# alexv879/ClusterMachineLearningForHospitalNetworks-Apache-Spark

Hardware: AMD Instinct MI355X
Metric: KMeans fit samples/sec (whole node), 100M×256 k=256 at 1/2/4/8 MI355X (higher is better)
Workload: dtype bf16; 1 GPU; model=KMeans k=256, 100000000x256, global_batch=100000000, parallelism=dp1, k=256, rows=100000000, dim=256

## Files before the change

### clustermachinelearningforhospitalnetworks_apache_spark_amd/_native/csrc/kmeans.hip

```cpp
#include <algorithm>

#include "common.h"

namespace {

constexpr int kAccumThreads = 1024;
constexpr int kSegThreads = 256;

template <int DP>
struct AssignShape {
  static constexpr int NCH = DP / 8;
  static constexpr int KS = DP >= 32 ? DP / 32 : 1;
};
constexpr int kAssignThreads = 512;

template <bool HI>
__device__ __forceinline__ unsigned f8x2_to_bf16x2(unsigned w) {
  typedef float f2 __attribute__((ext_vector_type(2)));
  const f2 v = __builtin_amdgcn_cvt_pk_f32_fp8((int)w, HI);
  return (__float_as_uint(v.x) >> 16) | (__float_as_uint(v.y) & 0xffff0000u);
}

template <int DP, bool F8>
__device__ __forceinline__ void load_x16(const void* __restrict__ Xv, long long n, long long ldx, long long row0,
// ... 512 lines not shown
      for (int u = 0; u < kScatterU; ++u) {
        rows[u] = (long long)b * grp + (q0 + (long long)u * per) * stride + o;
        lab[u] = rows[u] < n ? labels[rows[u]] : -1;
        rk[u] = rows[u] < n ? rank[rows[u]] : 0;
      }
#pragma unroll
      for (int u = 0; u < kScatterU; ++u)
        if (lab[u] >= 0) {
          const long long pos = (long long)soff[lab[u]] + rk[u];
          if (pos < n) perm[pos] = (int)rows[u];
        }
    }
  }
}

template <int CPL> struct RawCols;
template <> struct RawCols<2> { using T = unsigned; };
template <> struct RawCols<4> { using T = uint2; };
template <> struct RawCols<8> { using T = uint4; };

template <int CPL>
__device__ __forceinline__ void add_raw(double (&acc)[CPL], const typename RawCols<CPL>::T& w) {
  const unsigned* ws = reinterpret_cast<const unsigned*>(&w);
#pragma unroll
  for (int q = 0; q < CPL / 2; ++q) {
    acc[2 * q] += (double)bf16_to_f32((u16)(ws[q] & 0xffffu));
    acc[2 * q + 1] += (double)bf16_to_f32((u16)(ws[q] >> 16));
  }
}

template <int CPL>
__device__ __forceinline__ void add_raw_q(double (&acc)[CPL], const typename RawCols<CPL>::T& w, double qs,
                                          float qsf) {
  const unsigned* ws = reinterpret_cast<const unsigned*>(&w);
  if (qsf != 0.f) {
#pragma unroll
    for (int q = 0; q < CPL / 2; ++q) {
      acc[2 * q] += (double)rintf(bf16_to_f32((u16)(ws[q] & 0xffffu)) * qsf);
      acc[2 * q + 1] += (double)rintf(bf16_to_f32((u16)(ws[q] >> 16)) * qsf);
    }
  } else {
#pragma unroll
    for (int q = 0; q < CPL / 2; ++q) {
      acc[2 * q] += rint((double)bf16_to_f32((u16)(ws[q] & 0xffffu)) * qs);
      acc[2 * q + 1] += rint((double)bf16_to_f32((u16)(ws[q] >> 16)) * qs);
    }
  }
}

__device__ __forceinline__ float grid_scale_f32(double qs) {
  return (qs >= 0x1p-126 && qs <= 0x1p126) ? (float)qs : 0.f;
}

template <int CPL> struct RawCols8;
template <> struct RawCols8<4> { using T = unsigned; };
template <> struct RawCols8<8> { using T = uint2; };
template <> struct RawCols8<16> { using T = uint4; };

template <int CPL>
__device__ __forceinline__ void add_raw8(double (&acc)[CPL], const typename RawCols8<CPL>::T& w) {
  typedef float f2 __attribute__((ext_vector_type(2)));
  const unsigned* ws = reinterpret_cast<const unsigned*>(&w);
#pragma unroll
  for (int q = 0; q < CPL / 4; ++q) {
    const f2 a = __builtin_amdgcn_cvt_pk_f32_fp8((int)ws[q], false);
    const f2 b = __builtin_amdgcn_cvt_pk_f32_fp8((int)ws[q], true);
    acc[4 * q] += (double)a.x;
    acc[4 * q + 1] += (double)a.y;
    acc[4 * q + 2] += (double)b.x;
    acc[4 * q + 3] += (double)b.y;
  }
}

template <int CPL>
__device__ __forceinline__ void add_raw8_f32(float (&acc)[CPL], const typename RawCols8<CPL>::T& w) {
  typedef float f2 __attribute__((ext_vector_type(2)));
  const unsigned* ws = reinterpret_cast<const unsigned*>(&w);
#pragma unroll
  for (int q = 0; q < CPL / 4; ++q) {
    const f2 a = __builtin_amdgcn_cvt_pk_f32_fp8((int)ws[q], false);
    const f2 b = __builtin_amdgcn_cvt_pk_f32_fp8((int)ws[q], true);
    acc[4 * q] += a.x;
    acc[4 * q + 1] += a.y;
    acc[4 * q + 2] += b.x;
    acc[4 * q + 3] += b.y;
  }
}

template <int CPL, bool F8> struct SegRaw { using T = typename RawCols<CPL>::T; };
template <int CPL> struct SegRaw<CPL, true> { using T = typename RawCols8<CPL>::T; };

template <int CPL, bool F8>
__device__ __forceinline__ float sqdist_raw(const typename SegRaw<CPL, F8>::T& w, const float (&cv)[CPL]) {
  const unsigned* ws = reinterpret_cast<const unsigned*>(&w);
  float s = 0.f;
  if constexpr (F8) {
    typedef float f2 __attribute__((ext_vector_type(2)));
#pragma unroll
    for (int q = 0; q < CPL / 4; ++q) {
      const f2 a = __builtin_amdgcn_cvt_pk_f32_fp8((int)ws[q], false);
      const f2 b = __builtin_amdgcn_cvt_pk_f32_fp8((int)ws[q], true);
      const float e0 = a.x - cv[4 * q], e1 = a.y - cv[4 * q + 1], e2 = b.x - cv[4 * q + 2], e3 = b.y - cv[4 * q + 3];
      s = fmaf(e0, e0, s);
      s = fmaf(e1, e1, s);
      s = fmaf(e2, e2, s);
      s = fmaf(e3, e3, s);
    }
  } else {
#pragma unroll
    for (int q = 0; q < CPL / 2; ++q) {
      const float e0 = bf16_to_f32((u16)(ws[q] & 0xffffu)) - cv[2 * q];
      const float e1 = bf16_to_f32((u16)(ws[q] >> 16)) - cv[2 * q + 1];
      s = fmaf(e0, e0, s);
      s = fmaf(e1, e1, s);
    }
  }
  return s;
}

__device__ __forceinline__ float wave_total_dpp(float v) {
  v += __int_as_float(__builtin_amdgcn_update_dpp(0, __float_as_int(v), 0xB1, 0xf, 0xf, false));
  v += __int_as_float(__builtin_amdgcn_update_dpp(0, __float_as_int(v), 0x4E, 0xf, 0xf, false));
  v += __int_as_float(__builtin_amdgcn_update_dpp(0, __float_as_int(v), 0x141, 0xf, 0xf, false));
  v += __int_as_float(__builtin_amdgcn_update_dpp(0, __float_as_int(v), 0x140, 0xf, 0xf, false));
  v += __int_as_float(__builtin_amdgcn_update_dpp(0, __float_as_int(v), 0x142, 0xa, 0xf, false));
  v += __int_as_float(__builtin_amdgcn_update_dpp(0, __float_as_int(v), 0x143, 0xc, 0xf, false));
  return __int_as_float(__builtin_amdgcn_readlane(__float_as_int(v), 63));
}

__device__ __forceinline__ float batch16_totals(const float (&s)[16]) {
  const int lane = threadIdx.x & 63;
  const bool h5 = lane & 32, h4 = lane & 16, h3 = lane & 8, h2 = lane & 4;
  float a[8], b[4], c[2];
#pragma unroll
  for (int i = 0; i < 8; ++i) a[i] = (h5 ? s[8 + i] : s[i]) + __shfl_xor(h5 ? s[i] : s[8 + i], 32, 64);
#pragma unroll
  for (int i = 0; i < 4; ++i) b[i] = (h4 ? a[4 + i] : a[i]) + __shfl_xor(h4 ? a[i] : a[4 + i], 16, 64);
#pragma unroll
  for (int i = 0; i < 2; ++i) c[i] = (h3 ? b[2 + i] : b[i]) + __shfl_xor(h3 ? b[i] : b[2 + i], 8, 64);
  float v = (h2 ? c[1] : c[0]) + __shfl_xor(h2 ? c[0] : c[1], 4, 64);
  v += __int_as_float(__builtin_amdgcn_update_dpp(0, __float_as_int(v), 0xB1, 0xf, 0xf, false));
  v += __int_as_float(__builtin_amdgcn_update_dpp(0, __float_as_int(v), 0x4E, 0xf, 0xf, false));
  return __shfl(v, 4 * (lane & 15), 64);
}

struct SegUB {
  const u16* cb;
  long long ldc;
  float* ub;
  double qs;
  const float* cu = nullptr;
};

__device__ __forceinline__ long long seg_chunk(long long filled, long long waves) {
  const long long c = (filled + waves - 1) / waves;
  return c > 128 ? c : 128;
}

template <int CPL, bool F8, bool UB = false, bool Q = false>
__global__ __launch_bounds__(kSegThreads, (CPL <= 4 ? 4 : 1)) void kmeans_segacc(const void* __restrict__ X, long long n, long long ldx,
                                                             int Dp, int D, const int* __restrict__ perm,
                                                             const int* __restrict__ seg, int k,
                                                             double* __restrict__ msg, double* __restrict__ slots,
                                                             int* __restrict__ slot_c, const int* __restrict__ gate,
                                                             int want, SegUB sub) {
  using raw_t = typename SegRaw<CPL, F8>::T;
  constexpr int U = 16;
// ... 998 lines not shown
```

### clustermachinelearningforhospitalnetworks_apache_spark_amd/models/kmeans.py

```python
from __future__ import annotations

import math
import os
import types
from typing import List, Optional

import numpy as np
import torch

from .. import _native
from ..ops import kmeans_ops as K
from ..ops.group_ops import group_reduce
from ..parallel.comm import Communicator, local_comm
from ..utils import rng
from ..utils.device import padded_dim, round_up
from ..utils.fault import maybe_fail
from ..utils.trace import trace


def padded_dim_fp8(d: int) -> int:
    return max(256, 1 << max(0, (d - 1).bit_length()))


def to_device_matrix(x: torch.Tensor, d: Optional[int] = None) -> torch.Tensor:
# ... 906 lines not shown
        st.lb = torch.zeros(max(n, 1), dtype=torch.float32, device=dev)
        st.cb_old = torch.zeros_like(self.cb)
        st.cb_cost = torch.zeros_like(self.cb)
        st.cum = cum if lazy else None
        st.half_every = int(os.environ.get("CML_KMEANS_HALF_EVERY", "4"))
        st.replay = {} if os.environ.get("CML_KMEANS_REPLAY", "1") != "0" else None
        st.replay_refused = None
        st.pm_host = torch.zeros(1, dtype=torch.int32, pin_memory=True) if self.gpu else None
        self._pst = st
        if self._norms_ready:
            self._set_mx()
        lean = os.environ.get("CML_KMEANS_LEAN_STEP", "1") != "0" and not self.use_graph
        per_wg_all = -(-(-(-max(n, 1) // tr)) // ap.grid) * tr
        self.delta = K.DeltaState(max(n, 1), k, d, self.dp, 1, self.msg_len, dev, ap.grid, fp8=K.is_fp8(self.x),
                                  cap=max(st.cap_m, 1024), pcap=max(per_wg_all if lean else per_wg, 64), lean=lean)

    def _step_prune_dev(self) -> None:
        self._pdev_pre()
        self.comm.allreduce_async(self.msgs[0]).wait()
        self._pdev_post()

    def _pdev_pre(self) -> None:
        st, dl = self._pst, self.delta
        hint_full = int(st.pm_host[0]) != 0
        lean = dl.lean_step() and not hint_full
        if self._replay_ok():
            if self._replay(("pre", lean), lambda: self._pdev_pre_launches(lean)):
                dl.host_forced = False
                return
        self._pdev_pre_launches(lean)
# ... 20 lines not shown

    def _pdev_pre_launches(self, lean: bool) -> None:
        st, dl = self._pst, self.delta
        n, k, d, ap = self.n, self.k, self.d, self.aplan
        x, lab, msg = self.x, self.labels, self.msgs[0]
        K.prune_bounds_gated(lab[:n], st.ub, st.lb, st.drift, st.dmax, st.thr, st.c2, k, st.cand, st.count,
                             self.xnorm, st.cand_lab, st.cand_xn, st.flags, st.cum, st.pmode, st.cap_m,
                             st.backoff if st.nback > 0 else None, st.nback, st.ctr[0:1], mode_host=st.pm_host)
        K.assign_rr_ext(1, x, n, self.dp, self.cb, self.cnorm, ap, self.xnorm, lab, self.cost_part, st.ub, st.lb,
                        st.mc, st.tau, hist=self.hist, rank=self.rank, delta=dl, gate=st.pmode, want=1, cum=st.cum)
        K.assign_rr_ext(2, x, st.cap_m, self.dp, self.cb, self.cnorm, ap, st.cand_xn, lab, self.cost_part, st.ub,
                        st.lb, st.mc, st.tau, delta=dl, idx=st.cand, n_dev=st.count, lab_in=st.cand_lab,
                        gate=st.pmode, want=0, cum=st.cum)
        dl.gate(0, lean=lean)
        if not lean:
            K.accumulate_sort(x, n, self.dp, d, lab, self.rank, self.hist, ap, k, self.cost_part, self.off, self.seg,
                              self.perm, self.cplan, dl.acc[0], self.slots, gate=dl.mode[0], qscale=self._qscale)
        dl.accumulate(x, self.dp, lab, 0, self.cost_part, ap.grid, msg, qscale=self._qscale)

    def _replay_ok(self) -> bool:
        st = self._pst
        return (not self.use_graph and self._grid_done and st.replay is not None
                and not torch.cuda.is_current_stream_capturing())

    def _pdev_post(self) -> None:
        st = self._pst
        exact = self.use_graph or st.half_every <= 1 or self.iterations % st.half_every == 0
        if not (self._replay_ok() and not self.spherical and self.dp <= 2048
                and self._replay(("post", exact, self._conv_lim), lambda: self._pdev_post_launches(exact))):
            self._pdev_post_launches(exact)
        self._shift2 = self.shift2
        self._cost_fn = self._device_cost

# ... 31 lines not shown

    def _step_seeded(self) -> None:
        st, dl = self._pst, self.delta
        n, k, d, ap = self.n, self.k, self.d, self.aplan
        x, lab, msg = self.x, self.labels, self.msgs[0]
        if n:
            K.prune_bounds(lab, st.ub, st.lb, st.drift, st.dmax, st.thr, st.c2, k, st.cand, st.count,
                           xn=self.xnorm, cand_lab=st.cand_lab, cand_xn=st.cand_xn, zero_count=True, cum=st.cum)
            K.prune_gate(st.count, st.cap_m, st.flags, st.pmode)
            K.assign_rr_ext(1, x, n, self.dp, self.cb, self.cnorm, ap, self.xnorm, lab, self.cost_part, st.ub, st.lb,
                            st.mc, st.tau, hist=self.hist, rank=self.rank, delta=dl, gate=st.pmode, want=1,
                            cum=st.cum)
            K.assign_rr_ext(2, x, st.cap_m, self.dp, self.cb, self.cnorm, ap, st.cand_xn, lab, None, st.ub, st.lb,
                            st.mc, st.tau, delta=dl, idx=st.cand, n_dev=st.count, lab_in=st.cand_lab, gate=st.pmode,
                            want=0, cum=st.cum)
            K.label_hist(lab, n, ap, self.hist, self.rank, gate=st.pmode, want=0)
        self.cost_part.zero_()
        dl.invalidate()
        dl.gate(0)
        K.accumulate_sort(x, n, self.dp, d, lab, self.rank, self.hist, ap, k, self.cost_part, self.off, self.seg,
                          self.perm, self.cplan, dl.acc[0], self.slots, gate=dl.mode[0],
                          ub_centres=self.cb, ub=st.ub, qscale=self._qscale, cum=st.cum)
        dl.accumulate(x, self.dp, lab, 0, self.cost_part, ap.grid, msg, qscale=self._qscale)
        self.comm.allreduce_async(msg).wait()
        self._pdev_post()

    def _norms64(self) -> torch.Tensor:
        self._ensure_norms()
        if self._xnorm64 is None:
            self._xnorm64 = torch.empty(max(self.n, 1), dtype=torch.float64, device=self.device)
            if self.n:
                tmp = torch.empty(self.n, dtype=torch.float32, device=self.device)
                for _, r0, r1, xc in self._x_chunks(whole=True):
                    K.row_pass(xc, r1 - r0, self.dp, tmp[r0:r1], xn64=self._xnorm64[r0:r1])
        return self._xnorm64

    def _device_cost(self) -> torch.Tensor:
# ... 847 lines not shown
```

### clustermachinelearningforhospitalnetworks_apache_spark_amd/ops/kmeans_ops.py

```python
from __future__ import annotations

import ctypes
import os
import threading

from dataclasses import dataclass

import torch

from .. import _native
from .._native import c_dbl, c_int, c_ll, c_vp
from ..utils.device import LDS_BUDGET, num_cus, round_up

_native.register_kernel_sigs({
    "cml_kmeans_assign_lds_bytes": (c_ll, [c_int, c_int, c_int]),
    "cml_kmeans_assign_threads": (c_int, [c_int]),
    "cml_kmeans_set_assign_variant": (c_int, [c_int]),
    "cml_kmeans_assign_occupancy": (c_int, [c_int, c_int, c_int, c_int]),
    "cml_kmeans_seg_threads": (c_int, []),
    "cml_kmeans_seg_ints": (c_ll, [c_int]),
    "cml_kmeans_assign_bf16": (c_int, [c_vp, c_ll, c_ll, c_int, c_vp, c_ll, c_int, c_int, c_int, c_vp, c_vp, c_vp,
                                       c_vp, c_int, c_int, c_vp, c_vp, c_vp, c_int, c_int, c_vp, c_vp, c_vp, c_vp,
                                       c_int, c_int, c_vp]),
    "cml_kmeans_assign_rr_plan": (c_int, [c_int, c_int, c_int, c_int, c_vp]),
# ... 2 lines not shown
    "cml_kmeans_set_rr_m32": (c_int, [c_int]),
    "cml_kmeans_set_fp8_mx": (c_int, [c_int]),
    "cml_kmeans_assign_tile_rows": (c_int, [c_int]),
    "cml_row_sqnorm_bf16": (c_int, [c_vp, c_ll, c_ll, c_int, c_vp, c_vp]),
    "cml_row_sqnorm_fp8": (c_int, [c_vp, c_ll, c_ll, c_int, c_vp, c_vp]),
    "cml_kmeans_priv_lds_bytes": (c_ll, [c_int, c_int, c_int]),
    "cml_kmeans_accum_priv": (c_int, [c_vp, c_ll, c_ll, c_vp, c_int, c_int, c_int, c_int, c_vp, c_vp, c_int, c_int,
                                      c_vp]),
    "cml_kmeans_reduce": (c_int, [c_vp, c_vp, c_vp, c_int, c_int, c_int, c_int, c_int, c_vp, c_vp]),
    "cml_kmeans_sort_accum": (c_int, [c_vp, c_ll, c_ll, c_int, c_int, c_vp, c_vp, c_vp, c_int, c_int, c_int, c_int,
                                      c_vp, c_int, c_vp, c_vp, c_vp, c_int, c_int, c_vp, c_vp, c_vp, c_int, c_vp,
                                      ctypes.c_double, c_vp]),
    "cml_kmeans_sort_accum_ub": (c_int, [c_vp, c_ll, c_ll, c_int, c_int, c_vp, c_vp, c_vp, c_int, c_int, c_int,
                                         c_int, c_vp, c_int, c_vp, c_vp, c_vp, c_int, c_int, c_vp, c_vp, c_vp, c_int,
                                         c_vp, c_vp, c_ll, c_vp, ctypes.c_double, c_vp, c_vp]),
    "cml_kmeans_delta_gate": (c_int, [c_vp, c_int, c_int, c_vp, c_vp, c_vp, c_int, c_vp, c_vp]),
    "cml_kmeans_delta_accum": (c_int, [c_vp, c_ll, c_int, c_int, c_vp, c_vp, c_vp, c_vp, c_int, c_int, c_int, c_vp,
                                       c_int, c_vp, c_vp, c_vp, c_vp, c_int, c_int, c_vp, c_vp, c_vp, c_vp, c_vp,
                                       c_int, c_vp, c_int, ctypes.c_double, c_vp]),
    "cml_kmeans_seg_slot_doubles": (c_ll, [c_int, c_int]),
    "cml_kmeans_seg_slot_ints": (c_ll, [c_int]),
    "cml_kmeans_update": (c_int, [c_vp, c_int, c_ll, c_int, c_int, c_vp, c_vp, c_ll, c_int, c_int, c_vp, c_vp,
                                  ctypes.c_double, c_vp]),
    "cml_kmeans_prune_lower": (c_int, [c_vp, c_int, c_vp, c_vp, ctypes.c_float, ctypes.c_float, c_ll, c_vp, c_vp]),
    "cml_kmeans_prune_bounds": (c_int, [c_vp, c_vp, c_vp, c_vp, c_vp, c_vp, c_vp, c_int, c_ll, c_vp,
                                        c_vp, c_vp, c_vp, c_vp, c_vp, c_ll, c_vp, c_vp]),
    "cml_kmeans_prune_gate": (c_int, [c_vp, c_ll, c_vp, c_vp, c_vp, c_int, c_vp]),
    "cml_kmeans_converge_latch": (c_int, [c_vp, c_int, ctypes.c_double, c_vp, c_vp]),
    "cml_kmeans_cond_copy": (c_int, [c_vp, c_vp, c_ll, c_vp, c_vp, c_vp]),
    "cml_kmeans_seed_bounds": (c_int, [c_vp, c_vp, c_vp, c_vp, c_vp, c_vp, c_vp, c_vp, ctypes.c_float, c_ll,
# ... 485 lines not shown
    lib = _native.kernels()
    args = (x.data_ptr(), n, x.stride(0), dp, d, labels.data_ptr(), rank.data_ptr(), hist.data_ptr(), aplan.grid,
            aplan.round_rows, k, aplan.kp, cost_part.data_ptr(), aplan.grid, off.data_ptr(), seg.data_ptr(),
            perm.data_ptr(), plan.cpl, plan.seg_grid, msg.data_ptr(), slots[0].data_ptr(), slots[1].data_ptr(),
            int(is_fp8(x)), gate.data_ptr() if gate is not None else 0)
    if ub is not None:
        if ub_centres is None or ub_centres.dtype != torch.bfloat16 or ub.dtype != torch.float32 or ub.numel() < n:
            raise ValueError("accumulate_sort: ub needs bf16 centres and an f32 [n] output")
        status = lib.cml_kmeans_sort_accum_ub(*args, ub_centres.data_ptr(), ub_centres.stride(0), ub.data_ptr(),
                                              float(qscale), _ptr(cum), _native.stream_ptr(stream))
    else:
        status = lib.cml_kmeans_sort_accum(*args, float(qscale), _native.stream_ptr(stream))
    _native.check(status, "kmeans_sort_accum")


def sort_perm(labels: torch.Tensor, rank: torch.Tensor, hist: torch.Tensor, aplan: AssignPlan, n: int, k: int,
              off: torch.Tensor, seg: torch.Tensor, perm: torch.Tensor, tail: torch.Tensor | None = None,
              cost_part: torch.Tensor | None = None, stream=None) -> torch.Tensor:
    i32 = torch.int32
    if any(t.dtype != i32 or not t.is_contiguous() for t in (labels, rank, hist, off, seg, perm)):
        raise ValueError("sort_perm: contiguous int32 labels, rank, hist, off, seg and perm")
    if (labels.numel() < n or rank.numel() < n or perm.numel() < n or hist.numel() < aplan.grid * aplan.kp
            or off.numel() < k * aplan.grid or seg.numel() < seg_buffer_ints(k) or k > aplan.kp):
        raise ValueError("sort_perm: buffer lengths do not match n, k and the assign plan")
    if tail is None:
        tail = torch.empty(k + 1, dtype=torch.float64, device=labels.device)
    elif tail.dtype != torch.float64 or tail.numel() < k + 1 or not tail.is_contiguous():
        raise ValueError("sort_perm: tail is a contiguous f64 [k + 1] tensor")
    if cost_part is not None and (cost_part.dtype != torch.float64 or cost_part.numel() < aplan.grid):
        raise ValueError("sort_perm: cost_part is the assign's f64 [grid] tensor")
# ... 728 lines not shown
```

Baseline: 118.7 billion samples/s.

## Add row-block LDS bucketing accumulate kernel replacing global sort-based accumulate

Adds a new kmeans_blockacc kernel. Each workgroup takes a block of rows, counts their labels in LDS, bucket-sorts row indices locally, sums rows per centre into per-block f64 slabs, and optionally computes upper bounds in the same pass. This is meant to remove the global label histogram, sort and permutation passes of the sort-based accumulate. The trade-off is extra per-block slab storage and a reduction of those slabs, plus LDS pressure that limits occupancy. In auto mode it only runs when 80*k fits within the block row count, and the default path uses it for the upper-bound full accumulate while plain accumulates stay on the sort path unless the env var is set to 1.

After: 111.8 billion samples/s. 0.942x the previous value.

```diff
diff --git a/clustermachinelearningforhospitalnetworks_apache_spark_amd/_native/csrc/kmeans.hip b/clustermachinelearningforhospitalnetworks_apache_spark_amd/_native/csrc/kmeans.hip
--- a/clustermachinelearningforhospitalnetworks_apache_spark_amd/_native/csrc/kmeans.hip
+++ b/clustermachinelearningforhospitalnetworks_apache_spark_amd/_native/csrc/kmeans.hip
@@ -550,143 +550,9 @@
   }
 }
 
-template <int CPL> struct RawCols;
-template <> struct RawCols<2> { using T = unsigned; };
-template <> struct RawCols<4> { using T = uint2; };
-template <> struct RawCols<8> { using T = uint4; };
-
-template <int CPL>
-__device__ __forceinline__ void add_raw(double (&acc)[CPL], const typename RawCols<CPL>::T& w) {
-  const unsigned* ws = reinterpret_cast<const unsigned*>(&w);
-#pragma unroll
-  for (int q = 0; q < CPL / 2; ++q) {
-    acc[2 * q] += (double)bf16_to_f32((u16)(ws[q] & 0xffffu));
-    acc[2 * q + 1] += (double)bf16_to_f32((u16)(ws[q] >> 16));
-  }
-}
-
-template <int CPL>
-__device__ __forceinline__ void add_raw_q(double (&acc)[CPL], const typename RawCols<CPL>::T& w, double qs,
-                                          float qsf) {
-  const unsigned* ws = reinterpret_cast<const unsigned*>(&w);
-  if (qsf != 0.f) {
-#pragma unroll
-    for (int q = 0; q < CPL / 2; ++q) {
-      acc[2 * q] += (double)rintf(bf16_to_f32((u16)(ws[q] & 0xffffu)) * qsf);
-      acc[2 * q + 1] += (double)rintf(bf16_to_f32((u16)(ws[q] >> 16)) * qsf);
-    }
-  } else {
-#pragma unroll
-    for (int q = 0; q < CPL / 2; ++q) {
-      acc[2 * q] += rint((double)bf16_to_f32((u16)(ws[q] & 0xffffu)) * qs);
-      acc[2 * q + 1] += rint((double)bf16_to_f32((u16)(ws[q] >> 16)) * qs);
-    }
-  }
-}
-
-__device__ __forceinline__ float grid_scale_f32(double qs) {
-  return (qs >= 0x1p-126 && qs <= 0x1p126) ? (float)qs : 0.f;
-}
-
-template <int CPL> struct RawCols8;
-template <> struct RawCols8<4> { using T = unsigned; };
-template <> struct RawCols8<8> { using T = uint2; };
-template <> struct RawCols8<16> { using T = uint4; };
-
-template <int CPL>
-__device__ __forceinline__ void add_raw8(double (&acc)[CPL], const typename RawCols8<CPL>::T& w) {
-  typedef float f2 __attribute__((ext_vector_type(2)));
-  const unsigned* ws = reinterpret_cast<const unsigned*>(&w);
-#pragma unroll
-  for (int q = 0; q < CPL / 4; ++q) {
-    const f2 a = __builtin_amdgcn_cvt_pk_f32_fp8((int)ws[q], false);
-    const f2 b = __builtin_amdgcn_cvt_pk_f32_fp8((int)ws[q], true);
-    acc[4 * q] += (double)a.x;
-    acc[4 * q + 1] += (double)a.y;
-    acc[4 * q + 2] += (double)b.x;
-    acc[4 * q + 3] += (double)b.y;
-  }
-}
-
-template <int CPL>
-__device__ __forceinline__ void add_raw8_f32(float (&acc)[CPL], const typename RawCols8<CPL>::T& w) {
-  typedef float f2 __attribute__((ext_vector_type(2)));
-  const unsigned* ws = reinterpret_cast<const unsigned*>(&w);
-#pragma unroll
-  for (int q = 0; q < CPL / 4; ++q) {
-    const f2 a = __builtin_amdgcn_cvt_pk_f32_fp8((int)ws[q], false);
-    const f2 b = __builtin_amdgcn_cvt_pk_f32_fp8((int)ws[q], true);
-    acc[4 * q] += a.x;
-    acc[4 * q + 1] += a.y;
-    acc[4 * q + 2] += b.x;
-    acc[4 * q + 3] += b.y;
-  }
-}
-
-template <int CPL, bool F8> struct SegRaw { using T = typename RawCols<CPL>::T; };
-template <int CPL> struct SegRaw<CPL, true> { using T = typename RawCols8<CPL>::T; };
-
-template <int CPL, bool F8>
-__device__ __forceinline__ float sqdist_raw(const typename SegRaw<CPL, F8>::T& w, const float (&cv)[CPL]) {
-  const unsigned* ws = reinterpret_cast<const unsigned*>(&w);
-  float s = 0.f;
-  if constexpr (F8) {
-    typedef float f2 __attribute__((ext_vector_type(2)));
-#pragma unroll
-    for (int q = 0; q < CPL / 4; ++q) {
-      const f2 a = __builtin_amdgcn_cvt_pk_f32_fp8((int)ws[q], false);
-      const f2 b = __builtin_amdgcn_cvt_pk_f32_fp8((int)ws[q], true);
-      const float e0 = a.x - cv[4 * q], e1 = a.y - cv[4 * q + 1], e2 = b.x - cv[4 * q + 2], e3 = b.y - cv[4 * q + 3];
-      s = fmaf(e0, e0, s);
-      s = fmaf(e1, e1, s);
-      s = fmaf(e2, e2, s);
-      s = fmaf(e3, e3, s);
-    }
-  } else {
-#pragma unroll
-    for (int q = 0; q < CPL / 2; ++q) {
-      const float e0 = bf16_to_f32((u16)(ws[q] & 0xffffu)) - cv[2 * q];
-      const float e1 = bf16_to_f32((u16)(ws[q] >> 16)) - cv[2 * q + 1];
-      s = fmaf(e0, e0, s);
-      s = fmaf(e1, e1, s);
-    }
-  }
-  return s;
-}
-
-__device__ __forceinline__ float wave_total_dpp(float v) {
-  v += __int_as_float(__builtin_amdgcn_update_dpp(0, __float_as_int(v), 0xB1, 0xf, 0xf, false));
-  v += __int_as_float(__builtin_amdgcn_update_dpp(0, __float_as_int(v), 0x4E, 0xf, 0xf, false));
-  v += __int_as_float(__builtin_amdgcn_update_dpp(0, __float_as_int(v), 0x141, 0xf, 0xf, false));
-  v += __int_as_float(__builtin_amdgcn_update_dpp(0, __float_as_int(v), 0x140, 0xf, 0xf, false));
-  v += __int_as_float(__builtin_amdgcn_update_dpp(0, __float_as_int(v), 0x142, 0xa, 0xf, false));
-  v += __int_as_float(__builtin_amdgcn_update_dpp(0, __float_as_int(v), 0x143, 0xc, 0xf, false));
-  return __int_as_float(__builtin_amdgcn_readlane(__float_as_int(v), 63));
-}
-
-__device__ __forceinline__ float batch16_totals(const float (&s)[16]) {
-  const int lane = threadIdx.x & 63;
-  const bool h5 = lane & 32, h4 = lane & 16, h3 = lane & 8, h2 = lane & 4;
-  float a[8], b[4], c[2];
-#pragma unroll
-  for (int i = 0; i < 8; ++i) a[i] = (h5 ? s[8 + i] : s[i]) + __shfl_xor(h5 ? s[i] : s[8 + i], 32, 64);
-#pragma unroll
-  for (int i = 0; i < 4; ++i) b[i] = (h4 ? a[4 + i] : a[i]) + __shfl_xor(h4 ? a[i] : a[4 + i], 16, 64);
-#pragma unroll
-  for (int i = 0; i < 2; ++i) c[i] = (h3 ? b[2 + i] : b[i]) + __shfl_xor(h3 ? b[i] : b[2 + i], 8, 64);
-  float v = (h2 ? c[1] : c[0]) + __shfl_xor(h2 ? c[0] : c[1], 4, 64);
-  v += __int_as_float(__builtin_amdgcn_update_dpp(0, __float_as_int(v), 0xB1, 0xf, 0xf, false));
-  v += __int_as_float(__builtin_amdgcn_update_dpp(0, __float_as_int(v), 0x4E, 0xf, 0xf, false));
-  return __shfl(v, 4 * (lane & 15), 64);
-}
-
-struct SegUB {
-  const u16* cb;
-  long long ldc;
-  float* ub;
-  double qs;
-  const float* cu = nullptr;
-};
+}
+#include "kmeans_segsum.h"
+namespace {
 
 __device__ __forceinline__ long long seg_chunk(long long filled, long long waves) {
   const long long c = (filled + waves - 1) / waves;
diff --git a/clustermachinelearningforhospitalnetworks_apache_spark_amd/_native/csrc/kmeans_blockacc.hip b/clustermachinelearningforhospitalnetworks_apache_spark_amd/_native/csrc/kmeans_blockacc.hip
--- /dev/null
+++ b/clustermachinelearningforhospitalnetworks_apache_spark_amd/_native/csrc/kmeans_blockacc.hip
@@ -0,0 +1,427 @@
+#include "common.h"
+#include "kmeans_segsum.h"
+
+namespace {
+
+constexpr int kBlkThreads = 512;
+constexpr int kBlkWaves = kBlkThreads / 64;
+constexpr int kBlkMaxWaves = 16;
+constexpr int kBlkMaxRows = 65536;
+constexpr long long kBlkLdsLimit = 160 * 1024;
+
+int g_blk_rows = 32768;
+int g_blk_stage = 1;
+
+__host__ __device__ inline int blk_ki(int k) { return (k + 1 + 63) & ~63; }
+__host__ __device__ inline long long blk_head_bytes(int k) { return 4LL * (3 * blk_ki(k) + 2 * kBlkMaxWaves); }
+__host__ __device__ inline int blk_cap(int k, int B) { return (B + 15) / 16 * 16 + 16 * k; }
+__host__ __device__ inline long long blk_slab_stride(int k, int D, int B) {
+  return (long long)k * D + k + (long long)kBlkWaves * 1024 + (blk_cap(k, B) + 1) / 2;
+}
+__host__ __device__ inline long long blk_region_bytes(int k, int B, int cpl, int waves) {
+  const long long list = 2LL * blk_cap(k, B);
+  const long long part = 8LL * waves * 64 * cpl;
+  return ((list > part ? list : part) + 15) / 16 * 16;
+}
+inline int blk_threads(int cpl, bool stage) { return stage && cpl <= 4 ? 2 * kBlkThreads : kBlkThreads; }
+inline long long blk_lds_bytes(int k, int B, int cpl, bool stage) {
+  return blk_head_bytes(k) + blk_region_bytes(k, B, cpl, blk_threads(cpl, stage) / 64) +
+         (stage ? 2LL * ((B + 15) / 16 * 16) : 0);
+}
+
+template <int CPL, bool F8, bool UB, bool Q>
+__global__ __launch_bounds__((CPL <= 4 ? 2 : 1) * kBlkThreads, (CPL <= 4 ? 4 : 2)) void kmeans_blockacc(
+    const void* __restrict__ X, long long n, long long ldx, int Dp, int D, const int* __restrict__ labels, int k,
+    int B, int stage, double* slabs, const int* __restrict__ gate, int want, SegUB sub) {
+  using raw_t = typename SegRaw<CPL, F8>::T;
+  constexpr int U = 16;
+  constexpr int ESZ = F8 ? 1 : 2;
+  constexpr int DPART = 64 * CPL;
+  extern __shared__ __attribute__((aligned(16))) unsigned char blk_smem[];
+  if (gate != nullptr && gate[0] != want) return;
+  const int ki = blk_ki(k);
+  int* cnt = reinterpret_cast<int*>(blk_smem);
+  int* start = cnt + ki;
+  int* cur = start + ki;
+  int* wfc = cur + ki;
+  int* wtc = wfc + kBlkMaxWaves;
+  unsigned char* region = blk_smem + blk_head_bytes(k);
+  u16* list = reinterpret_cast<u16*>(region);
+  double* part = reinterpret_cast<double*>(region);
+  const unsigned char* xb = reinterpret_cast<const unsigned char*>(X);
+  const int tid = threadIdx.x, lane = tid & 63, wave = __builtin_amdgcn_readfirstlane(tid >> 6);
+  const int nthr = blockDim.x, nwav = nthr >> 6;
+  u16* inv = reinterpret_cast<u16*>(region + blk_region_bytes(k, B, CPL, nwav));
+  const int cap = blk_cap(k, B);
+  const long long kd = (long long)k * D;
+  double* slab = slabs + (long long)blockIdx.x * blk_slab_stride(k, D, B);
+  float* stg = reinterpret_cast<float*>(slab + kd + k + kBlkWaves * 1024);
+  const int col = CPL * lane;
+  const bool active = col < Dp;
+  double* hslot = slab + kd + k + wave * DPART + col;
+  for (long long i = tid; i < kd + k; i += nthr) slab[i] = 0.0;
+  const float qsf = grid_scale_f32(sub.qs);
+  float cv[CPL];
+  auto load_cv = [&](int cc) {
+#pragma unroll
+    for (int j = 0; j < CPL; ++j) cv[j] = active ? bf16_to_f32(sub.cb[(long long)cc * sub.ldc + col + j]) : 0.f;
+  };
+  auto ub_of = [](float s) { return sqrtf(s * (1.0f + 1.0f / 8192.0f)) * (1.0f + 1e-6f); };
+  auto ub_store = [&](float u, int cc) {
+    if (sub.cu == nullptr) return u;
+    const float cu = sub.cu[cc];
+    return (u - cu) + 1e-6f * (u + cu);
+  };
+  auto slab_add = [&](int cc, const double (&v)[CPL]) {
+    if (active) {
+      double* dst = slab + (long long)cc * D;
+#pragma unroll
+      for (int j = 0; j < CPL; ++j)
+        if (col + j < D) dst[col + j] += v[j];
+    }
+  };
+  auto uni = [](int v) { return __builtin_amdgcn_readfirstlane(v); };
+
+  const long long nblk = (n + B - 1) / B;
+  for (long long blk = blockIdx.x; blk < nblk; blk += gridDim.x) {
+    const long long row0 = blk * B;
+    const int nrows = (int)(n - row0 < (long long)B ? n - row0 : (long long)B);
+    for (int c = tid; c < ki; c += nthr) cnt[c] = 0;
+    __syncthreads();
+    const int* lb = labels + row0;
+    const int nv = (reinterpret_cast<uintptr_t>(lb) & 15) == 0 ? nrows >> 2 : 0;
+    auto for_labels = [&](auto&& f) {
+      for (int v0 = tid; v0 < nv; v0 += 4 * nthr) {
+        int4 q[4];
+#pragma unroll
+        for (int u = 0; u < 4; ++u) {
+          const int v = v0 + u * nthr;
+          q[u] = v < nv ? reinterpret_cast<const int4*>(lb)[v] : int4{-1, -1, -1, -1};
+        }
+#pragma unroll
+        for (int u = 0; u < 4; ++u) {
+          const int i = 4 * (v0 + u * nthr);
+          if (i < 4 * nv) {
+            f(i, q[u].x);
+            f(i + 1, q[u].y);
+            f(i + 2, q[u].z);
+            f(i + 3, q[u].w);
+          }
+        }
+      }
+      for (int i = 4 * nv + tid; i < nrows; i += nthr) f(i, lb[i]);
+    };
+    for_labels([&](int, int l) {
+      if ((unsigned)l < (unsigned)k) atomicAdd(&cnt[l], 1);
+    });
+    __syncthreads();
+    if (wave == 0) {
+      int carry = 0;
+      for (int base = 0; base < k; base += 64) {
+        const int c = base + lane;
+        const int v = c < k ? ((cnt[c] + 15) & ~15) : 0;
+        int incl = v;
+#pragma unroll
+        for (int o = 1; o < 64; o <<= 1) {
+          const int y = __shfl_up(incl, o, 64);
+          if (lane >= o) incl += y;
+        }
+        if (c < k) {
+          start[c] = carry + incl - v;
+          cur[c] = carry + incl - v;
+        }
+        carry += __shfl(incl, 63, 64);
+      }
+      if (lane == 0) start[k] = carry;
+    }
+    __syncthreads();
+    for (int c = tid; c < k; c += nthr) slab[kd + c] += (double)cnt[c];
+    for_labels([&](int i, int l) {
+      int p = 0xffff;
+      if ((unsigned)l < (unsigned)k) {
+        p = atomicAdd(&cur[l], 1);
+        if (p < cap) list[p] = (u16)i;
+        else p = 0xffff;
+      }
+      if constexpr (UB) {
+        if (stage) inv[i] = (u16)p;
+      }
+    });
+    __syncthreads();
+    const int nb = uni(start[k]) >> 4;
+    const int per = (nb + nwav - 1) / nwav;
+    const int b0 = wave * per;
+    const int b1 = b0 + per < nb ? b0 + per : nb;
+    int fc = -1, tc = -1, hc = -1, nflush = 0;
+    double acc[CPL];
+#pragma unroll
+    for (int j = 0; j < CPL; ++j) acc[j] = 0.0;
+    if (b0 < b1) {
+      const int pos0 = b0 << 4;
+      int lo = 0, hi = k;
+      while (hi - lo > 1) {
+        const int mid = (lo + hi) >> 1;
+        if (uni(start[mid]) <= pos0) lo = mid; else hi = mid;
+      }
+      int c = lo;
+      fc = c;
+      int next = uni(start[c + 1]);
+      int cend = uni(start[c]) + uni(cnt[c]);
+      if constexpr (UB) load_cv(c);
+      for (int b = b0; b < b1; ++b) {
+        const int pos = b << 4;
+        if (pos >= next) {
+          if (nflush == 0) {
+            if (active) {
+#pragma unroll
+              for (int j = 0; j < CPL; ++j) hslot[j] = acc[j];
+            }
+            hc = c;
+          } else {
+            slab_add(c, acc);
+          }
+          ++nflush;
+#pragma unroll
+          for (int j = 0; j < CPL; ++j) acc[j] = 0.0;
+          ++c;
+          while (uni(start[c + 1]) <= pos) ++c;
+          next = uni(start[c + 1]);
+          cend = uni(start[c]) + uni(cnt[c]);
+          if constexpr (UB) load_cv(c);
+        }
+        const int nreal = cend - pos < U ? cend - pos : U;
+        const int lid = lane < nreal ? (int)list[pos + lane] : 0;
+        raw_t w[U];
+#pragma unroll
+        for (int u = 0; u < U; ++u) {
+          const long long row = row0 + __builtin_amdgcn_readlane(lid, u);
+          if (u < nreal && active) {
+            w[u] = *reinterpret_cast<const raw_t*>(xb + (row * ldx + col) * ESZ);
+          } else {
+            w[u] = raw_t{};
+          }
+        }
+        if constexpr (UB) {
+          static_assert(U == 16, "batch16_totals");
+          float mine = 0.f;
+          if constexpr (CPL <= 8) {
+            float sq[U];
+#pragma unroll
+            for (int u = 0; u < U; ++u) sq[u] = sqdist_raw<CPL, F8>(w[u], cv);
+            mine = batch16_totals(sq);
+          } else {
+#pragma unroll
+            for (int u = 0; u < U; ++u) {
+              const float t = wave_total_dpp(sqdist_raw<CPL, F8>(w[u], cv));
+              mine = lane == u ? t : mine;
+            }
+          }
+          if (lane < nreal) {
+            const float v = ub_store(ub_of(mine), c);
+            if (stage) stg[pos + lane] = v;
+            else sub.ub[row0 + lid] = v;
+          }
+        }
+        if constexpr (F8) {
+          float p32[CPL];
+#pragma unroll
+          for (int j = 0; j < CPL; ++j) p32[j] = 0.f;
+#pragma unroll
+          for (int u = 0; u < U; ++u) add_raw8_f32<CPL>(p32, w[u]);
+#pragma unroll
+          for (int j = 0; j < CPL; ++j) acc[j] += (double)p32[j];
+        } else {
+#pragma unroll
+          for (int u = 0; u < U; ++u) {
+            if constexpr (Q) add_raw_q<CPL>(acc, w[u], sub.qs, qsf);
+            else add_raw<CPL>(acc, w[u]);
+          }
+        }
+      }
+      tc = c;
+    }
+    __syncthreads();
+    if (b0 < b1 && active) {
+#pragma unroll
+      for (int j = 0; j < CPL; ++j) part[wave * DPART + col + j] = acc[j];
+    }
+    if (lane == 0) {
+      wfc[wave] = fc;
+      wtc[wave] = tc;
+    }
+    __syncthreads();
+    if (b0 < b1) {
+      auto chain = [&](int w0, const double (&own)[CPL], double (&t)[CPL]) {
+#pragma unroll
+        for (int j = 0; j < CPL; ++j) t[j] = 0.0;
+        for (int v = w0; v < wave; ++v) {
+          if (active) {
+#pragma unroll
+            for (int j = 0; j < CPL; ++j) t[j] += part[v * DPART + col + j];
+          }
+        }
+#pragma unroll
+        for (int j = 0; j < CPL; ++j) t[j] += own[j];
+      };
+      double t[CPL];
+      if (nflush > 0) {
+        int w0 = wave;
+        while (w0 > 0 && uni(wtc[w0 - 1]) == hc) --w0;
+        double hacc[CPL];
+#pragma unroll
+        for (int j = 0; j < CPL; ++j) hacc[j] = active ? hslot[j] : 0.0;
+        chain(w0, hacc, t);
+        slab_add(hc, t);
+      }
+      const bool cont = wave + 1 < nwav && uni(wfc[wave + 1]) == tc;
+      if (!cont) {
+        int w0 = wave;
+        if (nflush == 0)
+          while (w0 > 0 && uni(wtc[w0 - 1]) == tc) --w0;
+        chain(w0, acc, t);
+        slab_add(tc, t);
+      }
+    }
+    if constexpr (UB) {
+      if (stage) {
+        for (int r0 = tid; r0 < nrows; r0 += 8 * nthr) {
+          float v[8];
+#pragma unroll
+          for (int q = 0; q < 8; ++q) {
+            const int r = r0 + q * nthr;
+            const int p = r < nrows ? (int)inv[r] : 0xffff;
+            v[q] = p != 0xffff ? __hip_atomic_load(&stg[p], __ATOMIC_RELAXED, __HIP_MEMORY_SCOPE_AGENT) : -1.f;
+          }
+#pragma unroll
+          for (int q = 0; q < 8; ++q) {
+            const int r = r0 + q * nthr;
+            if (r < nrows && inv[r] != 0xffff) sub.ub[row0 + r] = v[q];
+          }
+        }
+      }
+    }
+  }
+}
+
+__global__ __launch_bounds__(256) void kmeans_blockacc_reduce(const double* __restrict__ slabs, long long stride,
+                                                              int nwg, int k, int D,
+                                                              const double* __restrict__ cost_part, int ncost,
+                                                              double* __restrict__ msg, const int* __restrict__ gate,
+                                                              int want) {
+  if (gate != nullptr && gate[0] != want) return;
+  const long long len = (long long)k * D + k;
+  const long long idx = (long long)blockIdx.x * blockDim.x + threadIdx.x;
+  if (idx < len) {
+    double s = 0.0;
+    for (int g0 = 0; g0 < nwg; g0 += 8) {
+      double v[8];
+#pragma unroll
+      for (int q = 0; q < 8; ++q) v[q] = g0 + q < nwg ? slabs[(long long)(g0 + q) * stride + idx] : 0.0;
+#pragma unroll
+      for (int q = 0; q < 8; ++q) s += v[q];
+    }
+    msg[idx] = s;
+  } else if (idx == len) {
+    double cs = 0.0;
+    for (int i = 0; i < ncost; ++i) cs += cost_part[i];
+    msg[idx] = cs;
+  }
+}
+
+template <int CPL, bool F8, bool UB, bool Q>
+int launch_blockacc(const void* X, long long n, long long ldx, int Dp, int D, const int* labels, int k, int B,
+                    int stage, int grid, size_t lds, double* slabs, const int* gate, int want, SegUB sub,
+                    hipStream_t st) {
+  (void)hipFuncSetAttribute((const void*)kmeans_blockacc<CPL, F8, UB, Q>, hipFuncAttributeMaxDynamicSharedMemorySize,
+                      (int)lds);
+  hipLaunchKernelGGL((kmeans_blockacc<CPL, F8, UB, Q>), dim3(grid), dim3(blk_threads(CPL, UB && stage)), lds, st, X, n,
+                     ldx, Dp, D,
+                     labels, k, B, stage, slabs, gate, want, sub);
+  return cml_status();
+}
+
+bool blk_cpl_ok(int cpl, int Dp, int xfp8) {
+  const bool known = xfp8 ? (cpl == 4 || cpl == 8 || cpl == 16) : (cpl == 2 || cpl == 4 || cpl == 8);
+  return known && Dp >= 1 && 64 * cpl >= Dp;
+}
+
+bool blk_stage(int k, int B, int cpl) {
+  return g_blk_stage != 0 && blk_cap(k, B) < 0xffff && blk_lds_bytes(k, B, cpl, true) <= kBlkLdsLimit;
+}
+
+}
+
+CML_API int cml_kmeans_blockacc_rows() { return g_blk_rows; }
+CML_API int cml_kmeans_set_blockacc_rows(int b) {
+  if (b < 16 || b > kBlkMaxRows) return (int)hipErrorInvalidValue;
+  g_blk_rows = b;
+  return 0;
+}
+CML_API int cml_kmeans_set_blockacc_stage(int on) {
+  g_blk_stage = on != 0;
+  return 0;
+}
+CML_API long long cml_kmeans_blockacc_lds_bytes(int k, int cpl, int ub) {
+  return blk_lds_bytes(k, g_blk_rows, cpl, ub && blk_stage(k, g_blk_rows, cpl));
+}
+CML_API int cml_kmeans_blockacc_takes(int k, int Dp, int D, int cpl, int xfp8) {
+  return k >= 1 && D >= 1 && D <= Dp && blk_cpl_ok(cpl, Dp, xfp8) &&
+         blk_lds_bytes(k, g_blk_rows, cpl, false) <= kBlkLdsLimit;
+}
+CML_API int cml_kmeans_blockacc_per_cu(int k, int cpl, int xfp8, int ub) {
+  (void)xfp8;
+  const bool stage = ub && blk_stage(k, g_blk_rows, cpl);
+  const int by_regs = cpl <= 4 ? 2 * kBlkThreads / blk_threads(cpl, stage) : 1;
+  const long long lds = cml_kmeans_blockacc_lds_bytes(k, cpl, ub);
+  const int by_lds = lds > 0 ? (int)(kBlkLdsLimit / lds) : 0;
+  return by_lds < by_regs ? by_lds : by_regs;
+}
+CML_API long long cml_kmeans_blockacc_slab_doubles(int grid, int k, int D) {
+  return (long long)grid * blk_slab_stride(k, D, g_blk_rows);
+}
+
+CML_API int cml_kmeans_block_accum(const void* X, long long n, long long ldx, int Dp, int D, const int* labels, int k,
+                                   const double* cost_part, int ncost, int cpl, int grid, double* slabs,
+                                   long long slab_cap, double* msg, int xfp8, const int* gate, const void* cb,
+                                   long long ldc, float* ub, double qscale, const float* cu, void* stream) {
+  if (n < 0 || grid < 1 || ncost < 0 || ldx < Dp || slabs == nullptr || msg == nullptr || labels == nullptr ||
+      !cml_kmeans_blockacc_takes(k, Dp, D, cpl, xfp8))
+    return (int)hipErrorInvalidValue;
+  if ((cb == nullptr) != (ub == nullptr) || (ub != nullptr && ldc < Dp)) return (int)hipErrorInvalidValue;
+  hipStream_t st = (hipStream_t)stream;
+  const int want = 1;
+  const int B = g_blk_rows;
+  const long long nblk = (n + B - 1) / B;
+  const int wgs = (int)(nblk < grid ? nblk : grid);
+  const long long stride = blk_slab_stride(k, D, B);
+  if (wgs * stride > slab_cap) return (int)hipErrorInvalidValue;
+  const SegUB sub{(const u16*)cb, ldc, ub, qscale, cu};
+  if (wgs > 0) {
+    const int stage = ub != nullptr && blk_stage(k, B, cpl);
+    const size_t lds = (size_t)blk_lds_bytes(k, B, cpl, stage);
+    const bool q = !xfp8 && qscale != 0.0;
+    int e;
+#define CML_BLK_L(C, F, U, Q) \
+  launch_blockacc<C, F, U, Q>(X, n, ldx, Dp, D, labels, k, B, stage, wgs, lds, slabs, gate, want, sub, st)
+#define CML_BLK(C, F)                                                      \
+  if (ub != nullptr) {                                                     \
+    e = q ? CML_BLK_L(C, F, true, !F) : CML_BLK_L(C, F, true, false);     \
+  } else {                                                                 \
+    e = q ? CML_BLK_L(C, F, false, !F) : CML_BLK_L(C, F, false, false);   \
+  }
+    if (xfp8) {
+      if (cpl == 4) { CML_BLK(4, true) }
+      else if (cpl == 8) { CML_BLK(8, true) }
+      else { CML_BLK(16, true) }
+    } else if (cpl == 2) { CML_BLK(2, false) }
+    else if (cpl == 4) { CML_BLK(4, false) }
+    else { CML_BLK(8, false) }
+#undef CML_BLK
+#undef CML_BLK_L
+    if (e) return e;
+  }
+  const long long len = (long long)k * D + k + 1;
+  hipLaunchKernelGGL(kmeans_blockacc_reduce, dim3((unsigned)((len + 255) / 256)), dim3(256), 0, st, slabs, stride,
+                     wgs, k, D, cost_part, ncost, msg, gate, want);
+  return cml_status();
+}
diff --git a/clustermachinelearningforhospitalnetworks_apache_spark_amd/_native/csrc/kmeans_segsum.h b/clustermachinelearningforhospitalnetworks_apache_spark_amd/_native/csrc/kmeans_segsum.h
--- /dev/null
+++ b/clustermachinelearningforhospitalnetworks_apache_spark_amd/_native/csrc/kmeans_segsum.h
@@ -0,0 +1,144 @@
+#pragma once
+#include "common.h"
+
+namespace {
+
+template <int CPL> struct RawCols;
+template <> struct RawCols<2> { using T = unsigned; };
+template <> struct RawCols<4> { using T = uint2; };
+template <> struct RawCols<8> { using T = uint4; };
+
+template <int CPL>
+__device__ __forceinline__ void add_raw(double (&acc)[CPL], const typename RawCols<CPL>::T& w) {
+  const unsigned* ws = reinterpret_cast<const unsigned*>(&w);
+#pragma unroll
+  for (int q = 0; q < CPL / 2; ++q) {
+    acc[2 * q] += (double)bf16_to_f32((u16)(ws[q] & 0xffffu));
+    acc[2 * q + 1] += (double)bf16_to_f32((u16)(ws[q] >> 16));
+  }
+}
+
+template <int CPL>
+__device__ __forceinline__ void add_raw_q(double (&acc)[CPL], const typename RawCols<CPL>::T& w, double qs,
+                                          float qsf) {
+  const unsigned* ws = reinterpret_cast<const unsigned*>(&w);
+  if (qsf != 0.f) {
+#pragma unroll
+    for (int q = 0; q < CPL / 2; ++q) {
+      acc[2 * q] += (double)rintf(bf16_to_f32((u16)(ws[q] & 0xffffu)) * qsf);
+      acc[2 * q + 1] += (double)rintf(bf16_to_f32((u16)(ws[q] >> 16)) * qsf);
+    }
+  } else {
+#pragma unroll
+    for (int q = 0; q < CPL / 2; ++q) {
+      acc[2 * q] += rint((double)bf16_to_f32((u16)(ws[q] & 0xffffu)) * qs);
+      acc[2 * q + 1] += rint((double)bf16_to_f32((u16)(ws[q] >> 16)) * qs);
+    }
+  }
+}
+
+__device__ __forceinline__ float grid_scale_f32(double qs) {
+  return (qs >= 0x1p-126 && qs <= 0x1p126) ? (float)qs : 0.f;
+}
+
+template <int CPL> struct RawCols8;
+template <> struct RawCols8<4> { using T = unsigned; };
+template <> struct RawCols8<8> { using T = uint2; };
+template <> struct RawCols8<16> { using T = uint4; };
+
+template <int CPL>
+__device__ __forceinline__ void add_raw8(double (&acc)[CPL], const typename RawCols8<CPL>::T& w) {
+  typedef float f2 __attribute__((ext_vector_type(2)));
+  const unsigned* ws = reinterpret_cast<const unsigned*>(&w);
+#pragma unroll
+  for (int q = 0; q < CPL / 4; ++q) {
+    const f2 a = __builtin_amdgcn_cvt_pk_f32_fp8((int)ws[q], false);
+    const f2 b = __builtin_amdgcn_cvt_pk_f32_fp8((int)ws[q], true);
+    acc[4 * q] += (double)a.x;
+    acc[4 * q + 1] += (double)a.y;
+    acc[4 * q + 2] += (double)b.x;
+    acc[4 * q + 3] += (double)b.y;
+  }
+}
+
+template <int CPL>
+__device__ __forceinline__ void add_raw8_f32(float (&acc)[CPL], const typename RawCols8<CPL>::T& w) {
+  typedef float f2 __attribute__((ext_vector_type(2)));
+  const unsigned* ws = reinterpret_cast<const unsigned*>(&w);
+#pragma unroll
+  for (int q = 0; q < CPL / 4; ++q) {
+    const f2 a = __builtin_amdgcn_cvt_pk_f32_fp8((int)ws[q], false);
+    const f2 b = __builtin_amdgcn_cvt_pk_f32_fp8((int)ws[q], true);
+    acc[4 * q] += a.x;
+    acc[4 * q + 1] += a.y;
+    acc[4 * q + 2] += b.x;
+    acc[4 * q + 3] += b.y;
+  }
+}
+
+template <int CPL, bool F8> struct SegRaw { using T = typename RawCols<CPL>::T; };
+template <int CPL> struct SegRaw<CPL, true> { using T = typename RawCols8<CPL>::T; };
+
+template <int CPL, bool F8>
+__device__ __forceinline__ float sqdist_raw(const typename SegRaw<CPL, F8>::T& w, const float (&cv)[CPL]) {
+  const unsigned* ws = reinterpret_cast<const unsigned*>(&w);
+  float s = 0.f;
+  if constexpr (F8) {
+    typedef float f2 __attribute__((ext_vector_type(2)));
+#pragma unroll
+    for (int q = 0; q < CPL / 4; ++q) {
+      const f2 a = __builtin_amdgcn_cvt_pk_f32_fp8((int)ws[q], false);
+      const f2 b = __builtin_amdgcn_cvt_pk_f32_fp8((int)ws[q], true);
+      const float e0 = a.x - cv[4 * q], e1 = a.y - cv[4 * q + 1], e2 = b.x - cv[4 * q + 2], e3 = b.y - cv[4 * q + 3];
+      s = fmaf(e0, e0, s);
+      s = fmaf(e1, e1, s);
+      s = fmaf(e2, e2, s);
+      s = fmaf(e3, e3, s);
+    }
+  } else {
+#pragma unroll
+    for (int q = 0; q < CPL / 2; ++q) {
+      const float e0 = bf16_to_f32((u16)(ws[q] & 0xffffu)) - cv[2 * q];
+      const float e1 = bf16_to_f32((u16)(ws[q] >> 16)) - cv[2 * q + 1];
+      s = fmaf(e0, e0, s);
+      s = fmaf(e1, e1, s);
+    }
+  }
+  return s;
+}
+
+__device__ __forceinline__ float wave_total_dpp(float v) {
+  v += __int_as_float(__builtin_amdgcn_update_dpp(0, __float_as_int(v), 0xB1, 0xf, 0xf, false));
+  v += __int_as_float(__builtin_amdgcn_update_dpp(0, __float_as_int(v), 0x4E, 0xf, 0xf, false));
+  v += __int_as_float(__builtin_amdgcn_update_dpp(0, __float_as_int(v), 0x141, 0xf, 0xf, false));
+  v += __int_as_float(__builtin_amdgcn_update_dpp(0, __float_as_int(v), 0x140, 0xf, 0xf, false));
+  v += __int_as_float(__builtin_amdgcn_update_dpp(0, __float_as_int(v), 0x142, 0xa, 0xf, false));
+  v += __int_as_float(__builtin_amdgcn_update_dpp(0, __float_as_int(v), 0x143, 0xc, 0xf, false));
+  return __int_as_float(__builtin_amdgcn_readlane(__float_as_int(v), 63));
+}
+
+__device__ __forceinline__ float batch16_totals(const float (&s)[16]) {
+  const int lane = threadIdx.x & 63;
+  const bool h5 = lane & 32, h4 = lane & 16, h3 = lane & 8, h2 = lane & 4;
+  float a[8], b[4], c[2];
+#pragma unroll
+  for (int i = 0; i < 8; ++i) a[i] = (h5 ? s[8 + i] : s[i]) + __shfl_xor(h5 ? s[i] : s[8 + i], 32, 64);
+#pragma unroll
+  for (int i = 0; i < 4; ++i) b[i] = (h4 ? a[4 + i] : a[i]) + __shfl_xor(h4 ? a[i] : a[4 + i], 16, 64);
+#pragma unroll
+  for (int i = 0; i < 2; ++i) c[i] = (h3 ? b[2 + i] : b[i]) + __shfl_xor(h3 ? b[i] : b[2 + i], 8, 64);
+  float v = (h2 ? c[1] : c[0]) + __shfl_xor(h2 ? c[0] : c[1], 4, 64);
+  v += __int_as_float(__builtin_amdgcn_update_dpp(0, __float_as_int(v), 0xB1, 0xf, 0xf, false));
+  v += __int_as_float(__builtin_amdgcn_update_dpp(0, __float_as_int(v), 0x4E, 0xf, 0xf, false));
+  return __shfl(v, 4 * (lane & 15), 64);
+}
+
+struct SegUB {
+  const u16* cb;
+  long long ldc;
+  float* ub;
+  double qs;
+  const float* cu = nullptr;
+};
+
+}
diff --git a/clustermachinelearningforhospitalnetworks_apache_spark_amd/models/kmeans.py b/clustermachinelearningforhospitalnetworks_apache_spark_amd/models/kmeans.py
--- a/clustermachinelearningforhospitalnetworks_apache_spark_amd/models/kmeans.py
+++ b/clustermachinelearningforhospitalnetworks_apache_spark_amd/models/kmeans.py
@@ -944,6 +944,17 @@
         per_wg_all = -(-(-(-max(n, 1) // tr)) // ap.grid) * tr
         self.delta = K.DeltaState(max(n, 1), k, d, self.dp, 1, self.msg_len, dev, ap.grid, fp8=K.is_fp8(self.x),
                                   cap=max(st.cap_m, 1024), pcap=max(per_wg_all if lean else per_wg, 64), lean=lean)
+        self._bplan = self._bslab = None
+        self._bplain = False
+        bmode = os.environ.get("CML_KMEANS_BLOCKACC", "auto").lower()
+        if bmode not in ("auto", "0", "1"):
+            raise ValueError(f"CML_KMEANS_BLOCKACC={bmode!r}: auto, 0 or 1")
+        fp8 = K.is_fp8(self.x)
+        if (bmode != "0" and self._hs is None
+                and K.blockacc_takes(self.dp, d, k, self.cplan, fp8, auto=bmode == "auto")):
+            self._bplan = K.plan_block(max(n, 1), self.dp, d, k, self.cplan, dev.index or 0, fp8)
+            self._bslab = K.block_slabs(self._bplan, dev)
+            self._bplain = bmode == "1"
 
     def _step_prune_dev(self) -> None:
         self._pdev_pre()
@@ -994,9 +1005,19 @@
                         gate=st.pmode, want=0, cum=st.cum)
         dl.gate(0, lean=lean)
         if not lean:
-            K.accumulate_sort(x, n, self.dp, d, lab, self.rank, self.hist, ap, k, self.cost_part, self.off, self.seg,
-                              self.perm, self.cplan, dl.acc[0], self.slots, gate=dl.mode[0], qscale=self._qscale)
+            self._full_accumulate(x, n, lab)
         dl.accumulate(x, self.dp, lab, 0, self.cost_part, ap.grid, msg, qscale=self._qscale)
+
+    def _full_accumulate(self, x, n: int, lab, ub: bool = False) -> None:
+        st, dl = self._pst, self.delta
+        ubk = dict(ub_centres=self.cb, ub=st.ub, cum=st.cum) if ub else {}
+        if self._bplan is not None and (ub or self._bplain):
+            K.accumulate_block(x, n, self.dp, self.d, lab, self.k, self.cost_part, self._bplan, self._bslab,
+                               dl.acc[0], gate=dl.mode[0], qscale=self._qscale, **ubk)
+        else:
+            K.accumulate_sort(x, n, self.dp, self.d, lab, self.rank, self.hist, self.aplan, self.k, self.cost_part,
+                              self.off, self.seg, self.perm, self.cplan, dl.acc[0], self.slots, gate=dl.mode[0],
+                              qscale=self._qscale, **ubk)
 
     def _replay_ok(self) -> bool:
         st = self._pst
@@ -1058,13 +1079,12 @@
             K.assign_rr_ext(2, x, st.cap_m, self.dp, self.cb, self.cnorm, ap, st.cand_xn, lab, None, st.ub, st.lb,
                             st.mc, st.tau, delta=dl, idx=st.cand, n_dev=st.count, lab_in=st.cand_lab, gate=st.pmode,
                             want=0, cum=st.cum)
-            K.label_hist(lab, n, ap, self.hist, self.rank, gate=st.pmode, want=0)
+            if self._bplan is None:
+                K.label_hist(lab, n, ap, self.hist, self.rank, gate=st.pmode, want=0)
         self.cost_part.zero_()
         dl.invalidate()
         dl.gate(0)
-        K.accumulate_sort(x, n, self.dp, d, lab, self.rank, self.hist, ap, k, self.cost_part, self.off, self.seg,
-                          self.perm, self.cplan, dl.acc[0], self.slots, gate=dl.mode[0],
-                          ub_centres=self.cb, ub=st.ub, qscale=self._qscale, cum=st.cum)
+        self._full_accumulate(x, n, lab, ub=True)
         dl.accumulate(x, self.dp, lab, 0, self.cost_part, ap.grid, msg, qscale=self._qscale)
         self.comm.allreduce_async(msg).wait()
         self._pdev_post()
diff --git a/clustermachinelearningforhospitalnetworks_apache_spark_amd/ops/kmeans_ops.py b/clustermachinelearningforhospitalnetworks_apache_spark_amd/ops/kmeans_ops.py
--- a/clustermachinelearningforhospitalnetworks_apache_spark_amd/ops/kmeans_ops.py
+++ b/clustermachinelearningforhospitalnetworks_apache_spark_amd/ops/kmeans_ops.py
@@ -40,6 +40,15 @@
     "cml_kmeans_sort_accum_ub": (c_int, [c_vp, c_ll, c_ll, c_int, c_int, c_vp, c_vp, c_vp, c_int, c_int, c_int,
                                          c_int, c_vp, c_int, c_vp, c_vp, c_vp, c_int, c_int, c_vp, c_vp, c_vp, c_int,
                                          c_vp, c_vp, c_ll, c_vp, ctypes.c_double, c_vp, c_vp]),
+    "cml_kmeans_blockacc_rows": (c_int, []),
+    "cml_kmeans_set_blockacc_rows": (c_int, [c_int]),
+    "cml_kmeans_set_blockacc_stage": (c_int, [c_int]),
+    "cml_kmeans_blockacc_lds_bytes": (c_ll, [c_int, c_int, c_int]),
+    "cml_kmeans_blockacc_takes": (c_int, [c_int, c_int, c_int, c_int, c_int]),
+    "cml_kmeans_blockacc_per_cu": (c_int, [c_int, c_int, c_int, c_int]),
+    "cml_kmeans_blockacc_slab_doubles": (c_ll, [c_int, c_int, c_int]),
+    "cml_kmeans_block_accum": (c_int, [c_vp, c_ll, c_ll, c_int, c_int, c_vp, c_int, c_vp, c_int, c_int, c_int, c_vp,
+                                       c_ll, c_vp, c_int, c_vp, c_vp, c_ll, c_vp, ctypes.c_double, c_vp, c_vp]),
     "cml_kmeans_delta_gate": (c_int, [c_vp, c_int, c_int, c_vp, c_vp, c_vp, c_int, c_vp, c_vp]),
     "cml_kmeans_delta_accum": (c_int, [c_vp, c_ll, c_int, c_int, c_vp, c_vp, c_vp, c_vp, c_int, c_int, c_int, c_vp,
                                        c_int, c_vp, c_vp, c_vp, c_vp, c_int, c_int, c_vp, c_vp, c_vp, c_vp, c_vp,
@@ -555,6 +564,76 @@
     _native.check(status, "kmeans_sort_accum")
 
 
+@dataclass
+class BlockAccPlan:
+    cpl: int
+    grid: int
+    grid_ub: int
+    slab_doubles: int
+
+
+def blockacc_rows() -> int:
+    return int(_native.kernels().cml_kmeans_blockacc_rows())
+
+
+def set_blockacc_rows(b: int) -> None:
+    _native.check(_native.kernels().cml_kmeans_set_blockacc_rows(int(b)), "set_blockacc_rows")
+
+
+def set_blockacc_stage(on: bool) -> None:
+    _native.check(_native.kernels().cml_kmeans_set_blockacc_stage(int(bool(on))), "set_blockacc_stage")
+
+
+def blockacc_takes(dp: int, d: int, k: int, plan: AccumPlan, fp8: bool = False, auto: bool = False) -> bool:
+    if plan.mode != "sort" or k < 1:
+        return False
+    lib = _native.kernels()
+    if not lib.cml_kmeans_blockacc_takes(int(k), int(dp), int(d), int(plan.cpl), int(fp8)):
+        return False
+    if auto and (80 * k > blockacc_rows() or (fp8 and plan.cpl > 8)):
+        return False
+    return True
+
+
+def plan_block(n: int, dp: int, d: int, k: int, plan: AccumPlan, device_index: int = 0,
+               fp8: bool = False) -> BlockAccPlan:
+    if not blockacc_takes(dp, d, k, plan, fp8):
+        raise ValueError(f"row-block accumulate does not take dp={dp}, d={d}, k={k}")
+    lib = _native.kernels()
+    b = blockacc_rows()
+    nblk = (max(n, 1) + b - 1) // b
+    grids = [max(1, min(nblk, num_cus(device_index) * max(1, int(lib.cml_kmeans_blockacc_per_cu(
+        int(k), int(plan.cpl), int(fp8), ub))))) for ub in (0, 1)]
+    return BlockAccPlan(cpl=plan.cpl, grid=grids[0], grid_ub=grids[1],
+                        slab_doubles=int(lib.cml_kmeans_blockacc_slab_doubles(max(grids), k, d)))
+
+
+def block_slabs(bplan: BlockAccPlan, device) -> torch.Tensor:
+    return torch.empty(max(bplan.slab_doubles, 1), dtype=torch.float64, device=device)
+
+
+def accumulate_block(x: torch.Tensor, n: int, dp: int, d: int, labels: torch.Tensor, k: int,
+                     cost_part: torch.Tensor, bplan: BlockAccPlan, slabs: torch.Tensor, msg: torch.Tensor,
+                     stream=None, gate: torch.Tensor | None = None, ub_centres: torch.Tensor | None = None,
+                     ub: torch.Tensor | None = None, qscale: float = 0.0,
+                     cum: torch.Tensor | None = None) -> None:
+    if slabs.dtype != torch.float64 or slabs.numel() < bplan.slab_doubles or not slabs.is_contiguous():
+        raise ValueError("accumulate_block: slabs is the f64 scratch of block_slabs(bplan)")
+    if labels.dtype != torch.int32 or labels.numel() < n or msg.numel() < k * d + k + 1:
+        raise ValueError("accumulate_block: int32 labels [n] and an f64 message [k*d + k + 1]")
+    if (ub is None) != (ub_centres is None):
+        raise ValueError("accumulate_block: ub and ub_centres go together")
+    if ub is not None and (ub_centres.dtype != torch.bfloat16 or ub.dtype != torch.float32 or ub.numel() < n):
+        raise ValueError("accumulate_block: ub needs bf16 centres and an f32 [n] output")
+    status = _native.kernels().cml_kmeans_block_accum(
+        x.data_ptr(), n, x.stride(0), dp, d, labels.data_ptr(), k, cost_part.data_ptr(), cost_part.numel(),
+        bplan.cpl, bplan.grid if ub is None else bplan.grid_ub, slabs.data_ptr(), slabs.numel(), msg.data_ptr(),
+        int(is_fp8(x)), _ptr(gate), _ptr(ub_centres),
+        ub_centres.stride(0) if ub_centres is not None else 0, _ptr(ub), float(qscale), _ptr(cum),
+        _native.stream_ptr(stream))
+    _native.check(status, "kmeans_block_accum")
+
+
 def sort_perm(labels: torch.Tensor, rank: torch.Tensor, hist: torch.Tensor, aplan: AssignPlan, n: int, k: int,
               off: torch.Tensor, seg: torch.Tensor, perm: torch.Tensor, tail: torch.Tensor | None = None,
               cost_part: torch.Tensor | None = None, stream=None) -> torch.Tensor:
```
